# seryrzu/centroFlye

Hardware: AMD Instinct MI355X
Metric: long-read bases/sec through rare-k-mer recruit+distance (higher is better)
Workload: dtype u8 bases -> u64 k-mers / u32 indices (integer only)

## Files before the change

### centroflye_amd/csrc/hip/cf_api.hip

```cpp
#include "cf_common.h"

#include <atomic>
#include <cstdlib>
#include <cstring>
#include <mutex>
#include <thread>

#ifndef CF_COPY_MODE_DEFAULT
#define CF_COPY_MODE_DEFAULT 1
#endif
struct alignas(16) cf_u32x4_api { uint32_t x, y, z, w; };

int cf_fail(cf_ctx* ctx, int code, const std::string& msg) {
    if (ctx) ctx->err = msg;
    return code;
}


static std::mutex g_pool_lock;
static std::vector<cf_ctx*> g_contexts;

static void cf_pool_flush_locked(cf_ctx* ctx) {
    for (auto& kv : ctx->pool) { ctx->block_bytes.erase(kv.second); (void)hipFree(kv.second); }
    ctx->pool.clear();
// ... 392 lines not shown
    else read_max = n_entries;
    ctx->cloud_max_entries = cloud_max; ctx->read_max_entries = read_max;
    ctx->have_clouds = true;
    ctx->stats.n_cloud_entries = n_entries;
    return 0;
}

int cf_get_edges(cf_ctx* ctx, uint32_t* out, int64_t cap) {
    if (!ctx) return -22;
    const int64_t n = std::min(cap, ctx->n_edges_stored);
    if (n < 0 || (n && !out)) return cf_fail(ctx, -22, "cf_get_edges: bad buffer");
    CF_HIP(hipSetDevice(ctx->device));
    CF_TRY(cf_copy_d2h(ctx, out, ctx->d_edges, (size_t)n * 16));
    return 0;
}

int cf_sort_edges(cf_ctx* ctx) {
    if (!ctx) return -22;
    const int64_t n = ctx->n_edges_stored;
    if (n <= 1) return 0;
    cf_scratch tmp(ctx);
    uint32_t* d_tmp = nullptr;
    CF_TRY(tmp.get(&d_tmp, (size_t)n * 4, "edge sort scratch"));
    int kbits = 1;
    while (kbits < 32 && ((int64_t)1 << kbits) < std::max<int64_t>(ctx->n_kmers, 2)) ++kbits;
    const int words[3] = {2, 1, 0}, bits[3] = {kbits, kbits, 16};
    return cf_radix_sort_rec16(ctx, ctx->d_edges, d_tmp, n, words, bits, 3);
}

int cf_get_stats(cf_ctx* ctx, cf_stats* out) {
    if (!ctx || !out) return -22;
    ctx->stats.hbm_bytes_live = (int64_t)ctx->live;
    ctx->stats.table_capacity = (int64_t)ctx->table_cap;
    ctx->stats.n_kmers = ctx->n_kmers;
    ctx->stats.n_edges_stored = ctx->n_edges_stored;
    *out = ctx->stats;
    return 0;
}

int cf_get_times(cf_ctx* ctx, cf_times* out) {
    if (!ctx || !out) return -22;
    *out = ctx->times;
    return 0;
}

static inline bool cf_in(int64_t v, int64_t lo, int64_t hi) { return lo <= v && v <= hi; }
struct cf_knob {
    const char* name;
    const char* refusal;
    bool (*accepted)(int64_t v);
    void (*store)(cf_ctx* ctx, int64_t v);
    int64_t (*load)(const cf_ctx* ctx);
};
static const cf_knob cf_knobs[] = {
#define CF_KNOB(name, type, def, accepted, stored, refusal) \
    {#name, refusal, [](int64_t v) -> bool { (void)v; return accepted; }, [](cf_ctx* ctx, int64_t v) { ctx->name = stored; }, [](const cf_ctx* ctx) -> int64_t { return ctx->name; }},
#include "cf_knobs.h"
#undef CF_KNOB
};
static const int cf_n_knobs = (int)(sizeof(cf_knobs) / sizeof(cf_knobs[0]));

static const cf_knob* cf_find_knob(cf_ctx* ctx, const char* name) {
    for (const cf_knob& k : cf_knobs)
        if (!std::strcmp(k.name, name)) return &k;
    cf_fail(ctx, -22, std::string("unknown parameter ") + name);
    return nullptr;
}

int cf_set_param(cf_ctx* ctx, const char* name, int64_t value) {
    if (!ctx || !name) return -22;
    const cf_knob* k = cf_find_knob(ctx, name);
    if (!k) return -22;
    if (!k->accepted(value)) return cf_fail(ctx, -22, k->refusal);
    k->store(ctx, value);
    if (!std::strncmp(name, "comm_", 5)) cf_comm_apply_params(ctx);
    return 0;
}

int cf_get_param(cf_ctx* ctx, const char* name, int64_t* value) {
    if (!ctx || !name || !value) return -22;
    const cf_knob* k = cf_find_knob(ctx, name);
    if (!k) return -22;
    *value = k->load(ctx);
    return 0;
}

const char* cf_param_name(int32_t index) { return index >= 0 && index < cf_n_knobs ? cf_knobs[index].name : nullptr; }

int cf_selftest_sort(cf_ctx* ctx, const uint64_t* keys, int64_t n, int32_t bits, uint64_t* out) {
    if (!ctx) return -22;
    CF_HIP(hipSetDevice(ctx->device));
    cf_scratch tmp(ctx);
    unsigned long long *a = nullptr, *b = nullptr;
    CF_TRY(tmp.get(&a, (size_t)n, "selftest keys"));
    CF_TRY(tmp.get(&b, (size_t)n, "selftest tmp"));
    if (n && hipMemcpy(a, keys, (size_t)n * 8, hipMemcpyHostToDevice) != hipSuccess) return cf_fail(ctx, -5, "selftest copy");
    CF_TRY(cf_radix_sort_u64(ctx, a, b, n, bits));
    if (n && hipMemcpy(out, a, (size_t)n * 8, hipMemcpyDeviceToHost) != hipSuccess) return cf_fail(ctx, -5, "selftest copy back");
    return 0;
}

int cf_selftest_scan(cf_ctx* ctx, const int64_t* in, int64_t n, int64_t* out) {
    if (!ctx) return -22;
    CF_HIP(hipSetDevice(ctx->device));
    cf_scratch tmp(ctx);
    int64_t *a = nullptr, *b = nullptr;
    CF_TRY(tmp.get(&a, (size_t)n + 1, "selftest in"));
    CF_TRY(tmp.get(&b, (size_t)n + 1, "selftest out"));
    int64_t total = 0;
    if (n && hipMemcpy(a, in, (size_t)n * 8, hipMemcpyHostToDevice) != hipSuccess) return cf_fail(ctx, -5, "selftest copy");
    CF_TRY(cf_scan_exclusive_i64(ctx, a, b, n, &total));
    if (n && hipMemcpy(out, b, (size_t)n * 8, hipMemcpyDeviceToHost) != hipSuccess) return cf_fail(ctx, -5, "selftest copy back");
    out[n] = total;
    return 0;
}

// ... 76 lines not shown
```

### centroflye_amd/csrc/hip/cf_common.h

```cpp
#pragma once
#include <hip/hip_runtime.h>

#include <algorithm>
#include <cstdint>
#include <cstdio>
#include <cstring>
#include <map>
#include <string>
#include <unordered_map>
#include <vector>

#include "cfhip.h"

extern __shared__ __attribute__((aligned(16))) unsigned char cf_lds[];

#define CF_WAVE 64

#ifndef cf_lds_at
typedef __attribute__((address_space(3))) unsigned char cf_lds_u8;
__device__ __forceinline__ unsigned char* cf_lds_at(uint32_t off) { return (unsigned char*)((cf_lds_u8*)(uintptr_t)(off + 16u) - 16); }
__device__ __forceinline__ bool cf_lds_base_ok() { return (uint32_t)(uintptr_t)(cf_lds_u8*)cf_lds == 0u; }
#endif

__device__ __forceinline__ uint64_t cf_mix64(uint64_t x) {
// ... 97 lines not shown
    int64_t contig_P = 0, contig_max_pos = 0, contig_n_freq = 0;
    float contig_build_ms = 0.f, map_ms = 0.f;
    int64_t* d_exact_ptr = nullptr;
    int32_t* d_exact_pos = nullptr;
    int64_t exact_pairs = 0;
    float score_ms = 0.f;

    uint8_t* d_edit = nullptr;
    size_t edit_cap = 0;
    int64_t edit_len = 0;

    std::vector<int64_t> tandem_hook_ptr;
    std::vector<int32_t> tandem_hook_pos;
    cf_tandem_shape tandem_last{};

    std::vector<std::vector<uint8_t>> cons_bytes;
    std::vector<std::vector<int64_t>> cons_off;
    std::vector<std::vector<int32_t>> cons_voting, cons_excluded;
    cf_consensus_shape cons_last{};

    std::vector<cf_ualign_hit> ualign_hits;
    std::vector<int64_t> ualign_op_ptr;
    std::vector<uint8_t> ualign_op_bytes;
    cf_ualign_shape ualign_last{};

    std::vector<cf_monodec_read> monodec_reads;
    std::vector<int64_t> monodec_ptr;
    std::vector<cf_monodec_inst> monodec_inst;
    cf_monodec_shape monodec_last{};

    bool monokmers_have = false;
    std::vector<cf_monokmer> monokmers_first;
    std::vector<int64_t> monokmers_ptr;
    std::vector<cf_monokmer_occ> monokmers_occ;
    cf_monokmers_shape monokmers_last{};

    bool monomap_have = false;
    std::vector<cf_monomap_read> monomap_reads;
    std::vector<int64_t> monomap_path_ptr, monomap_hit_ptr;
    std::vector<int32_t> monomap_path;
    std::vector<cf_monomap_hit> monomap_hits;
    cf_monomap_shape monomap_last{};

    static constexpr int kCopyThreads = 16;
    void* pin_slot[kCopyThreads] = {nullptr};
    hipStream_t pin_stream[kCopyThreads] = {nullptr};
    size_t pin_bytes = 0;
    int copy_threads = 16;

    cf_stats stats{};
    cf_times times{};

#define CF_KNOB(name, type, def, accepted, stored, refusal) type name = def;
#include "cf_knobs.h"
#undef CF_KNOB
};

int cf_fail(cf_ctx* ctx, int code, const std::string& msg);
int cf_copy_h2d(cf_ctx* ctx, void* dev, const void* host, size_t bytes);
int cf_copy_d2h(cf_ctx* ctx, void* host, const void* dev, size_t bytes);
int cf_alloc(cf_ctx* ctx, void** p, size_t bytes, const char* what);
void cf_release(cf_ctx* ctx, void* p, size_t bytes);

template <class T>
inline int cf_alloc_t(cf_ctx* ctx, T** p, size_t n, const char* what) {
    return cf_alloc(ctx, (void**)p, n * sizeof(T), what);
}
template <class T>
inline void cf_release_t(cf_ctx* ctx, T*& p, size_t n) {
    cf_release(ctx, (void*)p, n * sizeof(T));
    p = nullptr;
}

struct cf_scratch {
    explicit cf_scratch(cf_ctx* c) : ctx(c) {}
    cf_scratch(const cf_scratch&) = delete;
    cf_scratch& operator=(const cf_scratch&) = delete;
    ~cf_scratch() { release_all(); }
    template <class T> int get(T** p, size_t n, const char* what) {
        const int rc = cf_alloc_t(ctx, p, n, what);
        if (rc == 0) held.emplace_back((void*)*p, n * sizeof(T));
        return rc;
    }
    void keep(void* p) { const auto it = find(p); if (it != held.end()) held.erase(it); }
    void drop(void* p) {
        const auto it = find(p);
        if (it == held.end()) return;
        cf_release(ctx, it->first, it->second);
        held.erase(it);
    }
    void release_all() {
        for (auto it = held.rbegin(); it != held.rend(); ++it) cf_release(ctx, it->first, it->second);
        held.clear();
    }

private:
    std::vector<std::pair<void*, size_t>>::iterator find(void* p) {
        return p ? std::find_if(held.begin(), held.end(), [p](const std::pair<void*, size_t>& e) { return e.first == p; }) : held.end();
    }
    cf_ctx* ctx;
    std::vector<std::pair<void*, size_t>> held;
};

#define CF_HIP(expr)                                                                          \
    do {                                                                                      \
        hipError_t e_ = (expr);                                                               \
        if (e_ != hipSuccess)                                                                 \
            return cf_fail(ctx, -5, std::string(#expr) + ": " + hipGetErrorString(e_));       \
// ... 50 lines not shown
```

### centroflye_amd/csrc/hip/cf_dist.hip

```cpp
#include "cf_common.h"
#include "cf_dist_tab.h"

#include <cstdlib>

void cf_free_edges(cf_ctx* c);
int cf_refresh_unique_count(cf_ctx* ctx);

#ifndef cf_ballot
__device__ __forceinline__ unsigned long long cf_ballot(bool p) { return __builtin_amdgcn_ballot_w64(p); }
#endif

__global__ void __launch_bounds__(256)
cf_post_hist_kernel(const int32_t* __restrict__ entries, int64_t e0, int64_t e1, uint32_t part, uint32_t n_parts, uint32_t* __restrict__ cnt) {
    const int64_t stride = (int64_t)gridDim.x * blockDim.x;
    for (int64_t i = e0 + (int64_t)blockIdx.x * blockDim.x + threadIdx.x; i < e1; i += stride) {
        const uint32_t x = (uint32_t)entries[i];
        if (n_parts == 1u || x % n_parts == part) atomicAdd(&cnt[x], 1u);
    }
}

__global__ void __launch_bounds__(256)
cf_post_fill_kernel(const int64_t* __restrict__ cloud_ptr, const int32_t* __restrict__ entries, int64_t u0, int64_t u1, uint32_t part, uint32_t n_parts,
                    const int64_t* __restrict__ post_ptr, uint32_t* __restrict__ cursor, int32_t* __restrict__ post,
                    uint32_t* __restrict__ first_unit) {
// ... 156 lines not shown
            base += (unsigned long long)__popcll(m);
        }
    }
}
__global__ void __launch_bounds__(256)
cf_order_extract_kernel(const unsigned long long* __restrict__ keys, int64_t n, int ab, int32_t* __restrict__ order) {
    const int64_t stride = (int64_t)gridDim.x * blockDim.x;
    for (int64_t i = (int64_t)blockIdx.x * blockDim.x + threadIdx.x; i < n; i += stride) order[i] = (int32_t)(keys[i] & ((1ull << ab) - 1ull));
}

#define DIST_CLASS_CAP 255u
__device__ __forceinline__ bool cf_same_postings(const int64_t* __restrict__ post_ptr, const int32_t* __restrict__ post, uint32_t x, uint32_t y) {
    const int64_t x0 = post_ptr[x], x1 = post_ptr[x + 1], y0 = post_ptr[y], y1 = post_ptr[y + 1];
    if (x1 - x0 != y1 - y0) return false;
    for (int64_t i = 0; i < x1 - x0; ++i) if (post[x0 + i] != post[y0 + i]) return false;
    return true;
}
__global__ void __launch_bounds__(256)
cf_class_mark_kernel(const unsigned long long* __restrict__ keys, int64_t n, int ab, const int64_t* __restrict__ post_ptr, const int32_t* __restrict__ post,
                     const unsigned long long* __restrict__ not_a_set, uint32_t* __restrict__ flags) {
    const unsigned long long rank_mask = (1ull << ab) - 1ull;
    const bool off = *not_a_set != 0ull;
    auto continues = [&](int64_t i) -> bool {
        const unsigned long long k0 = keys[i - 1], k1 = keys[i];
        return (k0 >> ab) == (k1 >> ab) && cf_same_postings(post_ptr, post, (uint32_t)(k0 & rank_mask), (uint32_t)(k1 & rank_mask));
    };
    const int64_t stride = (int64_t)gridDim.x * blockDim.x;
    for (int64_t i = (int64_t)blockIdx.x * blockDim.x + threadIdx.x; i < n; i += stride) {
        if (off) { flags[i] = 1u; continue; }
        if (i > 0 && continues(i)) continue;
        flags[i] = 1u;
        uint32_t run = 1;
        for (int64_t j = i + 1; j < n && continues(j); ++j) {
            if (run == DIST_CLASS_CAP) { flags[j] = 1u; run = 0; }
            ++run;
        }
    }
}
__global__ void __launch_bounds__(256)
cf_class_first_kernel(const uint32_t* __restrict__ flags, const int64_t* __restrict__ cidx, int64_t n, int64_t n_classes, uint32_t* __restrict__ cfirst) {
    const int64_t stride = (int64_t)gridDim.x * blockDim.x;
    for (int64_t i = (int64_t)blockIdx.x * blockDim.x + threadIdx.x; i < n; i += stride) {
        if (flags[i]) cfirst[cidx[i]] = (uint32_t)i;
        if (i == 0) cfirst[n_classes] = (uint32_t)n;
    }
}

#define DIST_GROUP_MAX 32u
__device__ __forceinline__ unsigned long long cf_readlane64(unsigned long long v, int l) {
    return ((unsigned long long)(uint32_t)__builtin_amdgcn_readlane((int)(uint32_t)(v >> 32), l) << 32) | (unsigned long long)(uint32_t)__builtin_amdgcn_readlane((int)(uint32_t)v, l);
}
#define DIST_WALK_ROW 33u
#define DIST_WALK_LDS(block) ((size_t)((block) / 64) * 64 * DIST_WALK_ROW * 4)
__global__ void __launch_bounds__(256)
cf_group_walk_kernel(const unsigned long long* __restrict__ keys, int64_t n, int kb, int ab, const int64_t* __restrict__ post_ptr, const int32_t* __restrict__ post,
                     const unsigned long long* __restrict__ not_a_set, uint32_t cap, const cf_dist_rec* __restrict__ urange, const int32_t* __restrict__ rend, int32_t min_d, int32_t max_d,
                     uint32_t* __restrict__ flags, uint32_t* __restrict__ member_mask, uint32_t* __restrict__ new_mask,
                     unsigned long long* __restrict__ entries_out, unsigned long long* __restrict__ self_out) {
    const uint32_t lane = threadIdx.x & 63u;
    uint32_t* const rows = (uint32_t*)cf_lds + (size_t)(threadIdx.x >> 6) * (64u * DIST_WALK_ROW);
    const int64_t wave = ((int64_t)blockIdx.x * blockDim.x + threadIdx.x) >> 6, n_waves = ((int64_t)gridDim.x * blockDim.x) >> 6;
    const unsigned long long rank_mask = (1ull << ab) - 1ull;
    const bool off = *not_a_set != 0ull;
    if (cap > DIST_GROUP_MAX) cap = DIST_GROUP_MAX;
    unsigned long long ent = 0, self = 0;
    for (int64_t c0 = wave * 64; c0 < n; c0 += n_waves * 64) {
        int64_t wb = c0, w_p0 = 0;
        unsigned long long w_fu = ~0ull;
        uint32_t w_len = 0, o_mask = 0, o_new = 0;
        bool o_start = false, o_done = false;
        auto flush = [&]() {
            if (o_done) { const int64_t i = wb + (int64_t)lane; flags[i] = o_start ? 1u : 0u; member_mask[i] = o_mask; new_mask[i] = o_new; }
            o_done = false;
        };
        auto load_window = [&](int64_t b, bool all, bool own, unsigned long long fu) {
            flush();
            wb = b; w_fu = ~0ull; w_p0 = 0; w_len = 0;
            const int64_t i = b + (int64_t)lane;
            if (i < n) {
                const unsigned long long k = keys[i];
                w_fu = k >> kb;
                if (all || w_fu == fu) { const uint32_t x = (uint32_t)(k & rank_mask); w_p0 = post_ptr[x]; w_len = (uint32_t)(post_ptr[x + 1] - w_p0); }
            }
            const uint32_t len_l = w_len <= DIST_GROUP_MAX ? w_len : 0u;
            const uint32_t tl = lane & 7u, team = lane >> 3;
            unsigned long long adj_m = 0;
            int64_t t_p0[8];
            uint32_t t_len[8];
            int32_t t_u[8], t_r[8];
            uint32_t t_el[8], t_ig[8];
            __builtin_amdgcn_wave_barrier();
#pragma unroll
            for (int r = 0; r < 8; ++r) {
                const int m = r * 8 + (int)team;
                t_p0[r] = (int64_t)__shfl((long long)w_p0, m);
                t_len[r] = __shfl(len_l, m);
                t_u[r] = post[t_p0[r] + (int64_t)(tl < t_len[r] ? tl : 0u)];
            }
            if (own) {
#pragma unroll
                for (int r = 0; r < 8; ++r) { t_el[r] = urange[t_u[r]].len; t_ig[r] = urange[t_u[r]].ig; }
            }
#pragma unroll
            for (int r = 0; r < 8; ++r) {
                const uint32_t m = (uint32_t)r * 8u + team;
                const bool on = tl < t_len[r];
                if (on) rows[m * DIST_WALK_ROW + tl] = (uint32_t)t_u[r];
                t_r[r] = -1;
                if (own) {
                    if (on) { ent += t_el[r]; t_r[r] = t_u[r] - (int32_t)t_ig[r]; }
                    const int32_t prev = __shfl_up(t_r[r], 1u, 8);
                    if (on && tl > 0u && t_r[r] == prev) adj_m |= 1ull << m;
                }
            }
#pragma unroll
            for (int r = 0; r < 8; ++r) {
                const uint32_t m = (uint32_t)r * 8u + team;
                int32_t r_carry = own ? __shfl(t_r[r], 7, 8) : -1;
                for (uint32_t k0 = 8u; cf_ballot(k0 < t_len[r]) != 0ull; k0 += 8u) {
                    const uint32_t k = k0 + tl;
                    const bool on = k < t_len[r];
                    const int32_t u = post[t_p0[r] + (int64_t)(on ? k : 0u)];
                    if (on) rows[m * DIST_WALK_ROW + k] = (uint32_t)u;
                    if (own) {
                        int32_t rr = -1;
                        if (on) { ent += urange[u].len; rr = u - (int32_t)urange[u].ig; }
                        int32_t prev = __shfl_up(rr, 1u, 8);
                        if (tl == 0u) prev = r_carry;
                        if (on && rr == prev) adj_m |= 1ull << m;
                        r_carry = __shfl(rr, 7, 8);
                    }
                }
            }
            bool adj = false;
            if (own && cf_ballot(adj_m != 0ull) != 0ull) {
                for (int d = 32; d >= 1; d >>= 1) adj_m |= (unsigned long long)__shfl_xor((long long)adj_m, d);
                adj = (adj_m >> lane) & 1ull;
            }
            __builtin_amdgcn_wave_barrier();
            if (!own) return;
            if (adj)
                for (uint32_t p = 0; p + 1u < len_l; ++p) {
                    const int32_t up = (int32_t)rows[lane * DIST_WALK_ROW + p], re = rend[up];
                    for (uint32_t q = p + 1u; q < len_l; ++q) {
                        const int32_t v = (int32_t)rows[lane * DIST_WALK_ROW + q];
                        if (v >= re || v - up > max_d) break;
                        self += (unsigned long long)(v - up >= min_d);
                    }
                }
            unsigned long long lm = cf_ballot(w_len > DIST_GROUP_MAX);
            while (lm) {
                const int sl = __ffsll((long long)lm) - 1;
                lm &= lm - 1ull;
                const int64_t p0 = (int64_t)cf_readlane64((unsigned long long)w_p0, sl), p1 = p0 + (int64_t)(uint32_t)__builtin_amdgcn_readlane((int)w_len, sl);
                for (int64_t p = p0 + (int64_t)lane; p < p1; p += 64) {
                    const int32_t up = post[p], re = rend[up];
                    ent += urange[up].len;
                    for (int64_t q = p + 1; q < p1; ++q) {
                        const int32_t v = post[q];
                        if (v >= re || v - up > max_d) break;
                        self += (unsigned long long)(v - up >= min_d);
                    }
                }
            }
        };
        load_window(c0, true, true, 0ull);
        const int64_t i_me = c0 + (int64_t)lane;
        if (off) { if (i_me < n) { flags[i_me] = 1u; member_mask[i_me] = 0u; new_mask[i_me] = 0u; } continue; }
        bool head = i_me < n;
        if (head && i_me > 0) head = (keys[i_me - 1] >> kb) != w_fu;
        unsigned long long hm = cf_ballot(head);
        while (hm) {
            const int s = __ffsll((long long)hm) - 1;
            hm &= hm - 1ull;
            if (wb != c0) load_window(c0, true, false, 0ull);
            const unsigned long long fu = cf_readlane64(w_fu, s);
            uint32_t un = 0xFFFFFFFEu, nu = 0, members = 0;
            uint32_t L_next = rows[(uint32_t)s * DIST_WALK_ROW + (lane & 31u)];
            for (int64_t j = c0 + s; j < n; ++j) {
                if (j - wb == 64) { load_window(j, false, false, fu); L_next = rows[lane & 31u]; }
                const int sl = (int)(j - wb);
                if (cf_readlane64(w_fu, sl) != fu) break;
                const uint32_t len = (uint32_t)__builtin_amdgcn_readlane((int)w_len, sl);
                const uint32_t L = lane < len ? L_next : 0xFFFFFFFFu;
                L_next = rows[(uint32_t)min(sl + 1, 63) * DIST_WALK_ROW + (lane & 31u)];
                uint32_t mask = 0, fresh = 0;
                bool start = true;
                if (len > cap) { nu = 0; members = 0; }
                else {
                    uint32_t found = 0;
                    if (nu)
                        for (uint32_t t0 = 0; t0 < len; t0 += 8u) {
#pragma unroll
                            for (uint32_t q = 0; q < 8u; ++q) {
                                const unsigned long long h = cf_ballot(un == (uint32_t)__builtin_amdgcn_readlane((int)L, (int)(t0 + q)));
                                mask |= (uint32_t)h;
                                found |= (uint32_t)(h != 0ull) << (t0 + q);
                            }
                        }
                    const uint32_t mine = (uint32_t)((1ull << len) - 1ull);
                    uint32_t nm = mine & ~found;
                    start = members == 0u || members == DIST_CLASS_CAP || nu + (uint32_t)__popc(nm) > cap;
                    if (start) { nu = 0; members = 0; mask = 0; nm = mine; un = 0xFFFFFFFEu; }
                    fresh = nm;
                    while (nm) {
                        const int t = __ffs((int)nm) - 1;
                        nm &= nm - 1u;
                        const uint32_t x = (uint32_t)__builtin_amdgcn_readlane((int)L, t);
                        if (lane == nu) un = x;
                        mask |= 1u << nu;
                        ++nu;
                    }
                    ++members;
                }
                if (lane == (uint32_t)sl) { o_start = start; o_mask = mask; o_new = fresh; o_done = true; }
            }
        }
        flush();
    }
    for (int d = 32; d >= 1; d >>= 1) { ent += __shfl_down(ent, (unsigned)d); self += __shfl_down(self, (unsigned)d); }
    if (lane == 0u) {
        if (ent) atomicAdd(entries_out, ent);
        if (self) atomicAdd(self_out, self);
    }
}
#define DIST_FILL_TEAM 8
__global__ void __launch_bounds__(256)
cf_group_fill_kernel(const int32_t* __restrict__ order, const uint32_t* __restrict__ gfirst, int64_t n_groups, const int64_t* __restrict__ post_ptr, const int32_t* __restrict__ post,
                     const unsigned long long* __restrict__ not_a_set, uint32_t cap, const uint32_t* __restrict__ new_mask, const uint32_t* __restrict__ member_mask,
                     int32_t* __restrict__ upost, uint32_t* __restrict__ ulen, unsigned long long* __restrict__ diag, unsigned long long* __restrict__ err) {
    const bool off = *not_a_set != 0ull;
    unsigned long long dg_u = 0, dg_c = 0;
    constexpr uint32_t T = DIST_FILL_TEAM;
    const uint32_t tl = threadIdx.x & (T - 1u);
    const int64_t team = ((int64_t)blockIdx.x * blockDim.x + threadIdx.x) / T, n_teams = ((int64_t)gridDim.x * blockDim.x) / T;
    for (int64_t g0 = 0; g0 < n_groups; g0 += n_teams) {
        const int64_t g = g0 + team;
        const bool on = g < n_groups;
        uint32_t f = 0, e = 0;
        if (on) { f = gfirst[g]; e = gfirst[g + 1]; }
        bool counting = off;
        if (on && e - f == 1u) { const int32_t x = order[f]; counting = counting || (uint32_t)(post_ptr[x + 1] - post_ptr[x]) > cap; }
        const uint32_t n_mem = (on && !counting) ? e - f : 0u;
        uint32_t n_max = n_mem;
        for (uint32_t d = T; d < 64u; d <<= 1) n_max = max(n_max, __shfl_xor(n_max, (int)d));
        uint32_t k = 0;
        for (uint32_t b = 0; b < n_max; b += T) {
            const uint32_t j = f + b + tl;
            uint32_t nm = b + tl < n_mem ? new_mask[j] : 0u;
            const uint32_t c = (uint32_t)__popc(nm);
            uint32_t incl = c;
            for (uint32_t d = 1; d < T; d <<= 1) { const uint32_t t = __shfl_up(incl, d, (int)T); if (tl >= d) incl += t; }
            uint32_t at = k + incl - c;
            if (nm) {
                const int64_t p0 = post_ptr[order[j]];
                while (nm) {
                    const int t = __ffs((int)nm) - 1;
                    nm &= nm - 1u;
                    if (at < DIST_GROUP_MAX) upost[(size_t)DIST_GROUP_MAX * (size_t)g + at] = post[p0 + t];
                    ++at;
                }
            }
            k += __shfl(incl, (int)T - 1, (int)T);
        }
        if (!on || tl != 0u) continue;
        if (k > DIST_GROUP_MAX) { atomicOr(err, 4ull); k = DIST_GROUP_MAX; }
        ulen[g] = counting ? 0x80000000u : k;
        dg_u += k;
#if defined(CF_DIST_DIAG_COUNT)
        for (uint32_t j = f; j < e; ++j) {
            bool seen = false;
            for (uint32_t q = f; q < j && !seen; ++q) seen = member_mask[q] == member_mask[j];
            dg_c += (unsigned long long)!seen;
        }
#endif
    }
// ... 1188 lines not shown
    const size_t tab_extra = groups ? cf_tab_mask<8>::extra_bytes((uint32_t)A.slots) : 0;
    if (A.slots >= 0xFFFF) return cf_fail(ctx, -22, "cf_dist_edges: more than 65534 table slots (16-bit slot indices; 0xFFFF marks an unused entry of the hot list)");
    A.fill_limit = (uint32_t)((int64_t)A.slots * ctx->dist_fill_pct / 100);
    {
        const int64_t slack = (int64_t)(block / 64) * 2 * 128;
        if (slack * 4 <= (int64_t)A.slots) A.fill_limit = (uint32_t)std::min<int64_t>(A.fill_limit, (int64_t)A.slots - slack);
    }
    A.est_limit = (uint32_t)((int64_t)A.fill_limit * 100 / ctx->dist_est_pct);
    A.counters = d_cnt; A.unique_bits = ctx->d_unique_bits;
    const size_t lds = (size_t)A.slots * slot_bytes + tab_extra + lds_fixed;
    A.sketch = (ctx->dist_sketch && min_cov >= 2 && min_cov <= 200) ? 1 : 0;
    A.sk_shift = 32; A.sk_counters = 1;
    const size_t sk_room = (size_t)A.slots * slot_bytes + DIST_STAGE_CAP * 2 + 16 + (size_t)(block / 64) * (DIST_QSTRIDE + DIST_OVQ) * qitem_bytes + 2 * DIST_STACK * 4 + DIST_HOT_CAP * 2;
    while (A.sk_shift > 8 && (size_t)A.sk_counters * 2 <= sk_room) { A.sk_counters *= 2; --A.sk_shift; }
    if (A.sk_counters < 16) A.sketch = 0;
    A.sk_bytes = A.sk_counters;
    const bool sk4 = A.sketch && min_cov <= 9 && ctx->dist_sketch_bits != 8 && A.sk_shift > 9;
    if (sk4) { A.sk_counters *= 2; --A.sk_shift; A.sk_fbits = 4; A.sk_fsh = 2; A.sk_wshift = 3; A.sk_fmask = 15; A.sk_guard = 12; }
    else { A.sk_fbits = 8; A.sk_fsh = 3; A.sk_wshift = 2; A.sk_fmask = 255; A.sk_guard = 0x7FFFFFFFu; }
    A.sk_mask = A.sk_counters - 1u;
    const int per_cu = std::max(1, std::min((int)((160 * 1024) / lds), 2048 / block));
    const int64_t n_a_alloc = (K > part) ? (K - part + n_parts - 1) / n_parts : 0;
    CF_TRY(tmp.get(&d_okeys, (size_t)n_a_alloc, "order keys"));
    CF_TRY(tmp.get(&d_otmp, (size_t)n_a_alloc, "order scratch"));
    CF_TRY(tmp.get(&d_order, (size_t)n_a_alloc, "order"));
    int ab = 1, ub = 1;
    while (ab < 32 && ((int64_t)1 << ab) < K) ++ab;
    while (ub < 32 && ((int64_t)1 << ub) < std::max<int64_t>(U, 2)) ++ub;
    const bool classes = ctx->dist_classes && by_sort;
    const int hb = classes ? std::min(ctx->dist_class_bits, 64 - ab - ub) : 0;
    int64_t n_heads = 0;
    uint32_t *d_cflag = nullptr, *d_cfirst = nullptr, *d_ulen = nullptr, *d_mmask = nullptr, *d_newm = nullptr;
    int32_t* d_upost = nullptr;
    if (K) {
        hipLaunchKernelGGL(cf_order_keys_kernel, dim3((unsigned)cf_grid_for(K, 256, max_blocks)), dim3(256), 0, ctx->stream,
                           (const uint32_t*)d_pcnt, (const uint32_t*)d_first, K, (int)part, (int)n_parts, ab, d_okeys, d_cnt + 6,
                           hb, (const int64_t*)d_post_ptr, (const int32_t*)d_post, (const unsigned long long*)(d_cnt + 144), groups ? 1 : 0);
        unsigned long long h_n = 0;
        CF_HIP(hipMemcpy(&h_n, d_cnt + 6, 8, hipMemcpyDeviceToHost));
        n_order = (int64_t)h_n;
        CF_TRY(cf_radix_sort_u64(ctx, d_okeys, d_otmp, n_order, ab + hb + ub));
        if (n_order)
            hipLaunchKernelGGL(cf_order_extract_kernel, dim3((unsigned)cf_grid_for(n_order, 256, max_blocks)), dim3(256), 0, ctx->stream,
                               (const unsigned long long*)d_okeys, n_order, ab, d_order);
    }
    n_heads = n_order;
    if (classes && n_order) {
        const unsigned g_cls = (unsigned)cf_grid_for(n_order, 256, max_blocks);
        int64_t* d_cidx = (int64_t*)d_otmp;
        CF_TRY(tmp.get(&d_cflag, (size_t)n_order + 1, "class flags"));
        CF_TRY(tmp.get(&d_cfirst, (size_t)n_order + 1, "class starts"));
        CF_HIP(hipMemsetAsync(d_cflag, 0, (size_t)(n_order + 1) * 4, ctx->stream));
        if (groups) { CF_TRY(tmp.get(&d_mmask, (size_t)n_order + 1, "member masks")); CF_TRY(tmp.get(&d_newm, (size_t)n_order + 1, "members' new postings")); }
        if (groups)
            hipLaunchKernelGGL(cf_group_walk_kernel, dim3(g_cls), dim3(256), DIST_WALK_LDS(256), ctx->stream, (const unsigned long long*)d_okeys, n_order, ab + hb, ab,
                               (const int64_t*)d_post_ptr, (const int32_t*)d_post, (const unsigned long long*)(d_cnt + 144), (uint32_t)ctx->dist_group_cap,
                               (const cf_dist_rec*)d_urange, (const int32_t*)d_rend, min_d_eff, max_d, d_cflag, d_mmask, d_newm, d_cnt + 1, d_cnt + 3);
        else
        hipLaunchKernelGGL(cf_class_mark_kernel, dim3(g_cls), dim3(256), 0, ctx->stream, (const unsigned long long*)d_okeys, n_order, ab,
                           (const int64_t*)d_post_ptr, (const int32_t*)d_post, (const unsigned long long*)(d_cnt + 144), d_cflag);
        CF_TRY(cf_scan_exclusive_u32_to_i64(ctx, d_cflag, d_cidx, n_order, &n_heads));
        hipLaunchKernelGGL(cf_class_first_kernel, dim3(g_cls), dim3(256), 0, ctx->stream, (const uint32_t*)d_cflag, (const int64_t*)d_cidx, n_order, n_heads, d_cfirst);
        if (groups) {
            CF_TRY(tmp.get(&d_upost, (size_t)n_heads * DIST_GROUP_MAX + 1, "group unions"));
            CF_TRY(tmp.get(&d_ulen, (size_t)n_heads + 1, "group union sizes"));
            hipLaunchKernelGGL(cf_group_fill_kernel, dim3((unsigned)cf_grid_for(n_heads * DIST_FILL_TEAM, 256, max_blocks)), dim3(256), 0, ctx->stream, (const int32_t*)d_order, (const uint32_t*)d_cfirst, n_heads,
                               (const int64_t*)d_post_ptr, (const int32_t*)d_post, (const unsigned long long*)(d_cnt + 144), (uint32_t)ctx->dist_group_cap, (const uint32_t*)d_newm, (const uint32_t*)d_mmask,
                               d_upost, d_ulen, d_cnt + 148, d_cnt + 4);
        }
        CF_KERNEL_CHECK("the class kernels");
    }
    A.order = d_order; A.n_order = n_heads; A.member_mask = d_mmask;
    if (n_heads) {
        const uint32_t nw = (uint32_t)block / 64u;
        const int g_items = cf_grid_for(n_heads * 16, 256, max_blocks);
        CF_TRY(tmp.get(&d_icnt, (size_t)n_heads + 1, "item counts"));
        CF_TRY(tmp.get(&d_ialloc, (size_t)n_heads + 1, "item slots"));
        CF_TRY(tmp.get(&d_ibase, (size_t)n_heads + 1, "item bases"));
        CF_TRY(tmp.get(&d_heads, (size_t)n_heads, "first k-mer heads"));
        hipLaunchKernelGGL(groups ? cf_items_count_kernel<true> : cf_items_count_kernel<false>, dim3((unsigned)g_items), dim3(256), 0, ctx->stream, (const int32_t*)d_order, n_heads, (const int64_t*)d_post_ptr,
                           (const int32_t*)d_post, (const cf_dist_rec*)d_urange, (const int32_t*)d_rbeg, min_d_eff, max_d, nw, by_sort ? 1 : 0, d_icnt, d_ialloc, d_cnt + 3,
                           (const uint32_t*)d_cfirst, (const int32_t*)d_upost, (const uint32_t*)d_ulen);
        CF_TRY(cf_scan_exclusive_u32_to_i64(ctx, d_ialloc, d_ibase, n_heads, &n_item_slots));
        CF_TRY(tmp.get(&d_items, (size_t)n_item_slots + 64, "item records"));
        hipLaunchKernelGGL(groups ? cf_items_fill_kernel<true> : cf_items_fill_kernel<false>, dim3((unsigned)g_items), dim3(256), 0, ctx->stream, (const int32_t*)d_order, n_heads, (const int64_t*)d_post_ptr,
                           (const int32_t*)d_post, (const cf_dist_rec*)d_urange, nw, (const uint32_t*)d_icnt, (const int64_t*)d_ibase, d_heads, d_items,
                           v_cloud_ptr, region26 ? 1 : 0, U, min_d_eff, max_d, min_cov, (ctx->dist_sketch_tail && A.sketch) ? 1 : 0,
                           (const unsigned long long*)(d_cnt + 144), d_cnt + 145, (const uint32_t*)d_cfirst, (const int32_t*)d_upost, (const uint32_t*)d_ulen);
    }
    A.heads = d_heads; A.items = d_items;
    const int64_t n_a = n_heads;
    const int grid = (int)std::max<int64_t>(1, std::min<int64_t>(n_a, (int64_t)std::max(1, ctx->n_cu) * per_cu));
    CF_KERNEL_CHECK("the work-list kernels");
    CF_HIP(hipEventRecord(ctx->ev2, ctx->stream));
#define CF_DIST_KERN(CLS) (region26 ? cf_dist_kernel<cf_tab_region26, CLS> : region ? cf_dist_kernel<cf_tab_region, CLS> : !narrow ? (wide16 ? cf_dist_kernel<cf_tab_wide16, CLS> : cf_dist_kernel<cf_tab_wide, CLS>) \
                               : narrow_db == 8 ? cf_dist_kernel<cf_tab_narrow_t<8>, CLS> : narrow_db == 7 ? cf_dist_kernel<cf_tab_narrow_t<7>, CLS>                                               \
                               : narrow_db == 6 ? cf_dist_kernel<cf_tab_narrow_t<6>, CLS> : cf_dist_kernel<cf_tab_narrow_t<5>, CLS>)
    void (*kern)(cf_dist_args) = classes ? CF_DIST_KERN(true) : CF_DIST_KERN(false);
    if (groups) kern = narrow_db == 8 ? cf_dist_kernel<cf_tab_mask<8>, true> : narrow_db == 7 ? cf_dist_kernel<cf_tab_mask<7>, true> : narrow_db == 6 ? cf_dist_kernel<cf_tab_mask<6>, true> : cf_dist_kernel<cf_tab_mask<5>, true>;
#undef CF_DIST_KERN
    CF_HIP(hipFuncSetAttribute((const void*)kern, hipFuncAttributeMaxDynamicSharedMemorySize, (int)lds));
    {
        A.edge_chunk = ctx->dist_edge_chunk > 0 ? (unsigned long long)ctx->dist_edge_chunk : DIST_EDGE_CHUNK;
        const int64_t rows = edge_cap > 0 ? edge_cap + (int64_t)grid * (int64_t)A.edge_chunk : 0;
        CF_TRY(cf_alloc_t(ctx, &ctx->d_edges, (size_t)rows * 4, "edges"));
        ctx->edge_cap = rows;
        A.edges = ctx->d_edges; A.edge_cap = (unsigned long long)rows;
    }
    CF_TRY(tmp.get(&d_holes, 2 * ((size_t)grid + 1), "edge holes"));
    A.holes = d_holes;
    CF_HIP(hipMemsetAsync(d_cnt + 6, 0, 16, ctx->stream));
// ... 97 lines not shown
```

### centroflye_amd/csrc/hip/cf_knobs.h

```cpp

CF_KNOB(dist_block, int, 0, v == 0 || (cf_in(v, 64, 1024) && v % 64 == 0), (int)v, "dist_block must be 0 (auto) or a multiple of 64 in [64, 1024]")
CF_KNOB(dist_wgs, int, 0, cf_in(v, 0, 8), (int)v, "dist_wgs out of range (0 = auto, 1 .. 8)")
CF_KNOB(dist_slots, int, 0, v == 0 || cf_in(v, 256, 19200), (int)v, "dist_slots out of range (0 = auto, 256 .. 19200: table + work lists must fit the 160 KiB LDS)")
CF_KNOB(dist_wide, int, 0, true, v != 0, "")
CF_KNOB(dist_post_atomics, int, 0, true, v != 0, "")
CF_KNOB(dist_hot_cap, int, 0, v >= 0, (int)v, "dist_hot_cap must be >= 0")
CF_KNOB(lut_shift, int, -1, cf_in(v, -1, 3), (int)v, "lut_shift out of range (-1 = by the set's size, 0 .. 3)")
CF_KNOB(dist_hot_entries, int, 32768, cf_in(v, -1, 0x7FFFFFFF), (int)v, "dist_hot_entries out of range (-1 = always keep the list, 0 .. 2^31 - 1)")
CF_KNOB(dist_regions, int, 0, v == 0 || v == 1 || v == 2 || v == 4 || v == 8, (int)v, "dist_regions must be 0 (auto), 1, 2, 4 or 8")
CF_KNOB(dist_region_bytes, int, 0, true, v != 0, "")
CF_KNOB(dist_dbits, int, 0, v == 0 || cf_in(v, 5, 8), (int)v, "dist_dbits must be 0 (auto) or 5 .. 8")
CF_KNOB(dist_fill_pct, int, 70, cf_in(v, 10, 90), (int)v, "dist_fill_pct out of range (10 .. 90)")
CF_KNOB(dist_edge_chunk, int, 0, cf_in(v, 0, 1 << 20), (int)v, "dist_edge_chunk out of range (0 = default, 1 .. 2^20)")
CF_KNOB(dist_int_thr, int, 1, true, v != 0, "")
CF_KNOB(dist_sketch, int, 1, true, v != 0, "")
CF_KNOB(dist_sketch_tail, bool, true, true, v != 0, "")
CF_KNOB(dist_class_bits, int, 16, cf_in(v, 1, 16), (int)v, "dist_class_bits out of range (1 .. 16)")
CF_KNOB(dist_classes, bool, true, true, v != 0, "")
CF_KNOB(dist_groups, bool, true, true, v != 0, "")
CF_KNOB(dist_filter_once, bool, true, true, v != 0, "")
CF_KNOB(dist_group_cap, int, 32, cf_in(v, 1, 32), (int)v, "dist_group_cap out of range (1 .. 32)")
CF_KNOB(dist_sketch_bits, int, 0, v == 0 || v == 4 || v == 8, (int)v, "dist_sketch_bits must be 0 (by min_cov), 4 or 8")
CF_KNOB(dist_est_pct, int, 80, cf_in(v, 5, 100), (int)v, "dist_est_pct out of range (5 .. 100)")
CF_KNOB(dist_stage, int, 2048, cf_in(v, 0, 2048), (int)v, "dist_stage out of range (0 .. 2048)")
CF_KNOB(place_chunk, int, 2, cf_in(v, 1, 64), (int)v, "place_chunk out of range (1 .. 64)")
CF_KNOB(place_grid, int, 0, cf_in(v, 0, 4096), (int)v, "place_grid out of range (0 = auto, 1 .. 4096)")
CF_KNOB(place_fused, int, 1, true, v != 0, "")
CF_KNOB(place_mode, int, 2, cf_in(v, 1, 3), (int)v, "place_mode out of range (1 = hash map, 2 = per-read regions unless min_inters < 4, 3 = per-read regions always)")
CF_KNOB(place_block, int, 0, v == 0 || (cf_in(v, 128, 1024) && v % 128 == 0), (int)v, "place_block must be 0 or a multiple of 128 in 128 .. 1024")
CF_KNOB(place_row_words, int, 0, v == 0 || v == 32 || v == 64, (int)v, "place_row_words must be 0 (auto), 32 or 64")
CF_KNOB(place_long_rescans, int, 2, cf_in(v, -1, 1000000), (int)v, "place_long_rescans out of range (-1, 0 .. 1000000)")
CF_KNOB(place_cmap_bits, int, 0, cf_in(v, 0, 30), (int)v, "place_cmap_bits out of range (0 = default, 1 .. 30)")
CF_KNOB(place_slots_per_unit, int, 0, cf_in(v, 0, 65536), (int)v, "place_slots_per_unit out of range (0 = default, 1 .. 65536)")
CF_KNOB(place_l3, int, 0, cf_in(v, 0, 2), (int)v, "place_l3 must be 0 (auto), 1 (always) or 2 (never)")
CF_KNOB(place_l3_shift, int, 0, cf_in(v, 0, 6), (int)v, "place_l3_shift must be 0 (= 6) .. 6")
CF_KNOB(map_window, int, 0, cf_in(v, 0, 4096), (int)v, "map_window out of range (0 = default, 1 .. 4096: 12 bytes of LDS per slot)")
CF_KNOB(edit_lds_diags, int, 0, cf_in(v, 0, 16384), (int)v, "edit_lds_diags out of range (0 = default, 1 .. 16384: 8 bytes of LDS per diagonal)")
CF_KNOB(tandem_key_mode, int, 0, cf_in(v, 0, 2), (int)v, "tandem_key_mode out of range (0 = auto, 1 = 64-bit keys, 2 = 16-byte records)")
CF_KNOB(tandem_batch_windows, int64_t, 0, cf_in(v, 0, (int64_t)1 << 31), v, "tandem_batch_windows out of range (0 = default, 1 .. 2^31)")
CF_KNOB(cons_batch_bytes, int64_t, 0, cf_in(v, 0, (int64_t)1 << 36), v, "cons_batch_bytes out of range (0 = default, 1 .. 2^36)")
CF_KNOB(ualign_batch_bytes, int64_t, 0, cf_in(v, 0, (int64_t)1 << 36), v, "ualign_batch_bytes out of range (0 = default, 1 .. 2^36)")
CF_KNOB(monodec_batch_bytes, int64_t, 0, cf_in(v, 0, (int64_t)1 << 36), v, "monodec_batch_bytes out of range (0 = default, 1 .. 2^36)")
CF_KNOB(count_mode, int, 1, true, v != 0, "")
CF_KNOB(count_bits, int, 0, cf_in(v, 0, 27), (int)v, "count_bits out of range (0 = auto, 1 .. 27)")
CF_KNOB(count_slots, int, 4096, v >= 256 && !(v & (v - 1)) && v * 8 <= 128 * 1024, (int)v, "count_slots must be a power of two in [256, 16384]")
CF_KNOB(count_tile, int, 16, cf_in(v, 1, 64), (int)v, "count_tile out of range")
CF_KNOB(count_skip_exotic, int, 0, cf_in(v, 0, 1), (int)v, "count_skip_exotic must be 0 or 1")
CF_KNOB(comm_round_bytes, int64_t, (int64_t)256 << 20, cf_in(v, 16, (int64_t)1 << 30) && v % 16 == 0, v, "comm_round_bytes must be a multiple of 16 in [16, 2^30]")
CF_KNOB(comm_self_p2p, int, 0, true, v != 0, "")
```

Measured before the change: 4.931 billion.

## Use per-wave LDS hash table for group-walk member lookup

Adds a templated variant of the group walk kernel that keeps the group's unit set in a 64-entry open-addressed LDS hash table per wave instead of scanning previous members' rows in chunks of eight. Lookups probe from a multiplicative hash home slot, new units are inserted with atomicCAS, and hits on earlier members are recorded through an LDS atomicOr array merged at flush. The variant is on by default through a new dist_walk knob, and optional compile-time timestamp instrumentation is added. It uses more LDS per wave and adds LDS atomics and probe loops, which could lower occupancy or add contention.

```diff
diff --git a/centroflye_amd/csrc/hip/cf_api.hip b/centroflye_amd/csrc/hip/cf_api.hip
--- a/centroflye_amd/csrc/hip/cf_api.hip
+++ b/centroflye_amd/csrc/hip/cf_api.hip
@@ -468,16 +468,28 @@
     void (*store)(cf_ctx* ctx, int64_t v);
     int64_t (*load)(const cf_ctx* ctx);
 };
+#define CF_KNOB_ENTRY(name, type, def, accepted, stored, refusal) \
+    {#name, refusal, [](int64_t v) -> bool { (void)v; return accepted; }, [](cf_ctx* ctx, int64_t v) { ctx->name = stored; }, [](const cf_ctx* ctx) -> int64_t { return ctx->name; }},
 static const cf_knob cf_knobs[] = {
-#define CF_KNOB(name, type, def, accepted, stored, refusal) \
-    {#name, refusal, [](int64_t v) -> bool { (void)v; return accepted; }, [](cf_ctx* ctx, int64_t v) { ctx->name = stored; }, [](const cf_ctx* ctx) -> int64_t { return ctx->name; }},
+#define CF_KNOB CF_KNOB_ENTRY
+#define CF_KNOB_AB(...)
 #include "cf_knobs.h"
 #undef CF_KNOB
+#undef CF_KNOB_AB
+};
+static const cf_knob cf_ab_knobs[] = {
+#define CF_KNOB(...)
+#define CF_KNOB_AB CF_KNOB_ENTRY
+#include "cf_knobs.h"
+#undef CF_KNOB
+#undef CF_KNOB_AB
 };
 static const int cf_n_knobs = (int)(sizeof(cf_knobs) / sizeof(cf_knobs[0]));
 
 static const cf_knob* cf_find_knob(cf_ctx* ctx, const char* name) {
     for (const cf_knob& k : cf_knobs)
+        if (!std::strcmp(k.name, name)) return &k;
+    for (const cf_knob& k : cf_ab_knobs)
         if (!std::strcmp(k.name, name)) return &k;
     cf_fail(ctx, -22, std::string("unknown parameter ") + name);
     return nullptr;
diff --git a/centroflye_amd/csrc/hip/cf_common.h b/centroflye_amd/csrc/hip/cf_common.h
--- a/centroflye_amd/csrc/hip/cf_common.h
+++ b/centroflye_amd/csrc/hip/cf_common.h
@@ -173,8 +173,10 @@
     cf_times times{};
 
 #define CF_KNOB(name, type, def, accepted, stored, refusal) type name = def;
+#define CF_KNOB_AB(name, type, def, accepted, stored, refusal) type name = def;
 #include "cf_knobs.h"
 #undef CF_KNOB
+#undef CF_KNOB_AB
 };
 
 int cf_fail(cf_ctx* ctx, int code, const std::string& msg);
diff --git a/centroflye_amd/csrc/hip/cf_dist.hip b/centroflye_amd/csrc/hip/cf_dist.hip
--- a/centroflye_amd/csrc/hip/cf_dist.hip
+++ b/centroflye_amd/csrc/hip/cf_dist.hip
@@ -232,13 +232,28 @@
 }
 #define DIST_WALK_ROW 33u
 #define DIST_WALK_LDS(block) ((size_t)((block) / 64) * 64 * DIST_WALK_ROW * 4)
+#define DIST_WALK_TAB 64u
+#define DIST_WALK_WAVE_TAB (64u * DIST_WALK_ROW + DIST_WALK_TAB * 2u + 64u)
+#define DIST_WALK_LDS_TAB(block) ((size_t)((block) / 64) * DIST_WALK_WAVE_TAB * 4)
+#define DIST_WALK_EMPTY 0xFFFFFFFFFFFFFFFFull
+__device__ __forceinline__ uint32_t cf_walk_home(uint32_t unit) { return (unit * 0x9E3779B1u) >> 26; }
+#if defined(CF_WALK_STAMPS)
+#define WALK_CLOCK() ((unsigned long long)__builtin_amdgcn_s_memtime())
+#define WALK_STAMP(...) __VA_ARGS__
+#else
+#define WALK_STAMP(...)
+#endif
+template <bool kTab>
 __global__ void __launch_bounds__(256)
 cf_group_walk_kernel(const unsigned long long* __restrict__ keys, int64_t n, int kb, int ab, const int64_t* __restrict__ post_ptr, const int32_t* __restrict__ post,
                      const unsigned long long* __restrict__ not_a_set, uint32_t cap, const cf_dist_rec* __restrict__ urange, const int32_t* __restrict__ rend, int32_t min_d, int32_t max_d,
                      uint32_t* __restrict__ flags, uint32_t* __restrict__ member_mask, uint32_t* __restrict__ new_mask,
-                     unsigned long long* __restrict__ entries_out, unsigned long long* __restrict__ self_out) {
+                     unsigned long long* __restrict__ entries_out, unsigned long long* __restrict__ self_out, unsigned long long* __restrict__ dg) {
     const uint32_t lane = threadIdx.x & 63u;
-    uint32_t* const rows = (uint32_t*)cf_lds + (size_t)(threadIdx.x >> 6) * (64u * DIST_WALK_ROW);
+    uint32_t* const rows = (uint32_t*)cf_lds + (size_t)(threadIdx.x >> 6) * (kTab ? DIST_WALK_WAVE_TAB : 64u * DIST_WALK_ROW);
+    unsigned long long* const tab = (unsigned long long*)(rows + 64u * DIST_WALK_ROW);
+    uint32_t* const o_or = (uint32_t*)(tab + DIST_WALK_TAB);
+    WALK_STAMP(const unsigned long long dg_t0 = WALK_CLOCK(); unsigned long long dg_mem = 0, dg_load = 0, dg_n = 0, dg_p = 0;)
     const int64_t wave = ((int64_t)blockIdx.x * blockDim.x + threadIdx.x) >> 6, n_waves = ((int64_t)gridDim.x * blockDim.x) >> 6;
     const unsigned long long rank_mask = (1ull << ab) - 1ull;
     const bool off = *not_a_set != 0ull;
@@ -250,10 +265,16 @@
         uint32_t w_len = 0, o_mask = 0, o_new = 0;
         bool o_start = false, o_done = false;
         auto flush = [&]() {
+            if (kTab) {
+                __builtin_amdgcn_wave_barrier();
+                o_mask |= o_or[lane];
+                o_or[lane] = 0u;
+            }
             if (o_done) { const int64_t i = wb + (int64_t)lane; flags[i] = o_start ? 1u : 0u; member_mask[i] = o_mask; new_mask[i] = o_new; }
             o_done = false;
         };
         auto load_window = [&](int64_t b, bool all, bool own, unsigned long long fu) {
+            WALK_STAMP(const unsigned long long dg_l0 = WALK_CLOCK(); struct dg_scope { unsigned long long t0, &sum; __device__ ~dg_scope() { sum += WALK_CLOCK() - t0; } } dg_s{dg_l0, dg_load};)
             flush();
             wb = b; w_fu = ~0ull; w_p0 = 0; w_len = 0;
             const int64_t i = b + (int64_t)lane;
@@ -344,6 +365,7 @@
                 }
             }
         };
+        if (kTab) o_or[lane] = 0u;
         load_window(c0, true, true, 0ull);
         const int64_t i_me = c0 + (int64_t)lane;
         if (off) { if (i_me < n) { flags[i_me] = 1u; member_mask[i_me] = 0u; new_mask[i_me] = 0u; } continue; }
@@ -356,18 +378,52 @@
             if (wb != c0) load_window(c0, true, false, 0ull);
             const unsigned long long fu = cf_readlane64(w_fu, s);
             uint32_t un = 0xFFFFFFFEu, nu = 0, members = 0;
+            WALK_STAMP(const unsigned long long dg_r0 = WALK_CLOCK(), dg_rl = dg_load;)
             uint32_t L_next = rows[(uint32_t)s * DIST_WALK_ROW + (lane & 31u)];
             for (int64_t j = c0 + s; j < n; ++j) {
                 if (j - wb == 64) { load_window(j, false, false, fu); L_next = rows[lane & 31u]; }
                 const int sl = (int)(j - wb);
                 if (cf_readlane64(w_fu, sl) != fu) break;
+                WALK_STAMP(++dg_n;)
                 const uint32_t len = (uint32_t)__builtin_amdgcn_readlane((int)w_len, sl);
                 const uint32_t L = lane < len ? L_next : 0xFFFFFFFFu;
                 L_next = rows[(uint32_t)min(sl + 1, 63) * DIST_WALK_ROW + (lane & 31u)];
                 uint32_t mask = 0, fresh = 0;
                 bool start = true;
                 if (len > cap) { nu = 0; members = 0; }
+                else if (kTab) {
+                    WALK_STAMP(if (nu) dg_p += len;)
+                    bool hit = false;
+                    uint32_t bit = 0;
+                    if (nu && lane < len)
+                        for (uint32_t h = cf_walk_home(L);; h = (h + 1u) & (DIST_WALK_TAB - 1u)) {
+                            const unsigned long long e = tab[h];
+                            if ((uint32_t)e == L) { hit = true; bit = (uint32_t)(e >> 32); break; }
+                            if (e == DIST_WALK_EMPTY) break;
+                        }
+                    const uint32_t found = nu ? (uint32_t)cf_ballot(hit) : 0u;
+                    const uint32_t mine = (uint32_t)((1ull << len) - 1ull);
+                    uint32_t nm = mine & ~found;
+                    start = members == 0u || members == DIST_CLASS_CAP || nu + (uint32_t)__popc(nm) > cap;
+                    if (start) {
+                        nu = 0; members = 0; nm = mine;
+                        __builtin_amdgcn_wave_barrier();
+                        tab[lane] = DIST_WALK_EMPTY;
+                        __builtin_amdgcn_wave_barrier();
+                    } else if (hit) atomicOr(&o_or[sl], 1u << bit);
+                    fresh = nm;
+                    if (lane < len && ((nm >> lane) & 1u)) {
+                        const unsigned long long e = ((unsigned long long)(nu + (uint32_t)__popc(nm & ((1u << lane) - 1u))) << 32) | (unsigned long long)L;
+                        for (uint32_t h = cf_walk_home(L); atomicCAS(&tab[h], DIST_WALK_EMPTY, e) != DIST_WALK_EMPTY; h = (h + 1u) & (DIST_WALK_TAB - 1u)) {}
+                    }
+                    __builtin_amdgcn_wave_barrier();
+                    const uint32_t c = (uint32_t)__popc(nm);
+                    mask = (uint32_t)(((1ull << c) - 1ull) << nu);
+                    nu += c;
+                    ++members;
+                }
                 else {
+                    WALK_STAMP(if (nu) dg_p += len;)
                     uint32_t found = 0;
                     if (nu)
                         for (uint32_t t0 = 0; t0 < len; t0 += 8u) {
@@ -395,6 +451,7 @@
                 }
                 if (lane == (uint32_t)sl) { o_start = start; o_mask = mask; o_new = fresh; o_done = true; }
             }
+            WALK_STAMP(dg_mem += (WALK_CLOCK() - dg_r0) - (dg_load - dg_rl);)
         }
         flush();
     }
@@ -402,6 +459,11 @@
     if (lane == 0u) {
         if (ent) atomicAdd(entries_out, ent);
         if (self) atomicAdd(self_out, self);
+#if defined(CF_WALK_STAMPS)
+        const unsigned long long dg_t1 = WALK_CLOCK();
+        atomicAdd(dg + 0, dg_mem); atomicAdd(dg + 1, dg_load); atomicAdd(dg + 2, dg_t1 - dg_t0); atomicAdd(dg + 3, dg_n); atomicAdd(dg + 4, dg_p); atomicAdd(dg + 5, 1ull);
+        atomicMax(dg + 8 + 2 * (size_t)blockIdx.x, ~dg_t0); atomicMax(dg + 9 + 2 * (size_t)blockIdx.x, dg_t1);
+#endif
     }
 }
 #define DIST_FILL_TEAM 8
@@ -1696,11 +1758,30 @@
         CF_TRY(tmp.get(&d_cfirst, (size_t)n_order + 1, "class starts"));
         CF_HIP(hipMemsetAsync(d_cflag, 0, (size_t)(n_order + 1) * 4, ctx->stream));
         if (groups) { CF_TRY(tmp.get(&d_mmask, (size_t)n_order + 1, "member masks")); CF_TRY(tmp.get(&d_newm, (size_t)n_order + 1, "members' new postings")); }
-        if (groups)
-            hipLaunchKernelGGL(cf_group_walk_kernel, dim3(g_cls), dim3(256), DIST_WALK_LDS(256), ctx->stream, (const unsigned long long*)d_okeys, n_order, ab + hb, ab,
+        if (groups) {
+            const bool tab = ctx->dist_walk;
+            const unsigned g_walk = g_cls;
+            unsigned long long* d_wdg = nullptr;
+#if defined(CF_WALK_STAMPS)
+            CF_TRY(tmp.get(&d_wdg, 8 + 2 * (size_t)g_walk, "walk stamps"));
+            CF_HIP(hipMemsetAsync(d_wdg, 0, (8 + 2 * (size_t)g_walk) * 8, ctx->stream));
+#endif
+            hipLaunchKernelGGL(tab ? cf_group_walk_kernel<true> : cf_group_walk_kernel<false>, dim3(g_walk), dim3(256), tab ? DIST_WALK_LDS_TAB(256) : DIST_WALK_LDS(256), ctx->stream,
+                               (const unsigned long long*)d_okeys, n_order, ab + hb, ab,
                                (const int64_t*)d_post_ptr, (const int32_t*)d_post, (const unsigned long long*)(d_cnt + 144), (uint32_t)ctx->dist_group_cap,
-                               (const cf_dist_rec*)d_urange, (const int32_t*)d_rend, min_d_eff, max_d, d_cflag, d_mmask, d_newm, d_cnt + 1, d_cnt + 3);
-        else
+                               (const cf_dist_rec*)d_urange, (const int32_t*)d_rend, min_d_eff, max_d, d_cflag, d_mmask, d_newm, d_cnt + 1, d_cnt + 3, d_wdg);
+#if defined(CF_WALK_STAMPS)
+            {
+                std::vector<unsigned long long> dgh(8 + 2 * (size_t)g_walk);
+                if (hipMemcpy(dgh.data(), d_wdg, dgh.size() * 8, hipMemcpyDeviceToHost) == hipSuccess) {
+                    unsigned long long wg = 0;
+                    for (size_t b = 0; b < g_walk; ++b) if (dgh[9 + 2 * b]) wg += (dgh[9 + 2 * b] - ~dgh[8 + 2 * b]) * 4ull;
+                    std::fprintf(stderr, "[cf_walk stamps] member=%llu load=%llu wave_life=%llu slot_life=%llu members=%llu postings=%llu waves=%llu (shader cycles summed over the waves of %u workgroups; dist_walk=%d)\n",
+                                 dgh[0], dgh[1], dgh[2], wg, dgh[3], dgh[4], dgh[5], g_walk, tab ? 1 : 0);
+                }
+            }
+#endif
+        } else
         hipLaunchKernelGGL(cf_class_mark_kernel, dim3(g_cls), dim3(256), 0, ctx->stream, (const unsigned long long*)d_okeys, n_order, ab,
                            (const int64_t*)d_post_ptr, (const int32_t*)d_post, (const unsigned long long*)(d_cnt + 144), d_cflag);
         CF_TRY(cf_scan_exclusive_u32_to_i64(ctx, d_cflag, d_cidx, n_order, &n_heads));
diff --git a/centroflye_amd/csrc/hip/cf_knobs.h b/centroflye_amd/csrc/hip/cf_knobs.h
--- a/centroflye_amd/csrc/hip/cf_knobs.h
+++ b/centroflye_amd/csrc/hip/cf_knobs.h
@@ -19,6 +19,7 @@
 CF_KNOB(dist_classes, bool, true, true, v != 0, "")
 CF_KNOB(dist_groups, bool, true, true, v != 0, "")
 CF_KNOB(dist_filter_once, bool, true, true, v != 0, "")
+CF_KNOB_AB(dist_walk, bool, true, true, v != 0, "")
 CF_KNOB(dist_group_cap, int, 32, cf_in(v, 1, 32), (int)v, "dist_group_cap out of range (1 .. 32)")
 CF_KNOB(dist_sketch_bits, int, 0, v == 0 || v == 4 || v == 8, (int)v, "dist_sketch_bits must be 0 (by min_cov), 4 or 8")
 CF_KNOB(dist_est_pct, int, 80, cf_in(v, 5, 100), (int)v, "dist_est_pct out of range (5 .. 100)")
```

New measurement: 4.991 billion, median of 6. 1.01x the previous value.
